# DonsetPG/graph-physics

Measured on AMD Instinct MI355X. Metric: training steps/sec, CylinderFlow 15-round MGN (batch 16 meshes per step), higher is better.
Workload: dtype f32; 1 GPU; BASELINE.json configs[1], fp32: 16 x 1885-node CylinderFlow-like meshes per GPU (N=30160, E=180082), 15 rounds, latent 128, random init; global_batch_meshes=16, launch=eager, parallelism=single

## Files before the change

graph-physics_amd/_capi.py:

```python
from __future__ import annotations

import ctypes as C
import os
import subprocess
import threading

_HERE = os.path.dirname(os.path.abspath(__file__))
_CSRC = os.path.join(_HERE, "csrc")
_REPO = os.path.dirname(_HERE)
LIB_PATH = os.environ.get("MGN_LIB") or os.path.join(_CSRC, "libmgn_hip.so")
SOURCES = [os.path.join(_CSRC, "mgn_kernels.hip"), os.path.join(_CSRC, "mgn_prep.hip"), os.path.join(_CSRC, "mgn_attn.hip"),
           os.path.join(_CSRC, "mgn_dense.hip"), os.path.join(_CSRC, "mgn_loss.hip"), os.path.join(_CSRC, "mgn_khop.hip"),
           os.path.join(_CSRC, "mgn_subgraph.hip"), os.path.join(_CSRC, "mgn_randedge.hip"), os.path.join(_CSRC, "mgn_knn.hip")]
DEPS = [os.path.join(_CSRC, "mgn_x6.inc"), os.path.join(_CSRC, "mgn_fused.inc"), os.path.join(_CSRC, "mgn_pp.inc"), os.path.join(_CSRC, "mgn_ppr.inc"),
        os.path.join(_CSRC, "mgn_philox.inc"), os.path.join(_CSRC, "mgn_host.inc"), os.path.join(_CSRC, "mgn_graphprim.inc"),
        os.path.join(_CSRC, "mgn_rollout.inc"), os.path.join(_CSRC, "mgn_starattn.inc"),
        os.path.join(_CSRC, "mgn_slice.inc")]
HEADER = os.path.join(_REPO, "include", "mgn_hip.h")
EXT_HEADER = os.path.join(_REPO, "include", "mgn_hip_ext.h")
MTP_HEADER = os.path.join(_REPO, "include", "mgn_hip_mtp.h")
SLICE_HEADER = os.path.join(_REPO, "include", "mgn_hip_slice.h")
DEVICE_FLAGS = ["-Xclang", "-target-feature", "-Xclang", "-packed-fp32-ops"]

MAX_LAYERS = 8
# ... 4 lines not shown
_i32p = C.c_void_p


class MlpFwdArgs(C.Structure):
    _fields_ = [
        ("M", C.c_int64),
        ("H", C.c_int), ("NL", C.c_int), ("nphase", C.c_int),
        ("src", _f32p * MAX_PHASES),
        ("idx", _i32p * MAX_PHASES),
        ("kw", C.c_int * MAX_PHASES),
        ("W", _f32p * MAX_LAYERS),
        ("b", _f32p * MAX_LAYERS),
        ("scale", _f32p),
        ("eps", C.c_float),
        ("out_w", C.c_int),
        ("resid", _f32p),
        ("out", _f32p),
        ("y_out", _f32p),
        ("saveH", _f32p * MAX_LAYERS),
        ("saveU", _f32p),
        ("saveR", _f32p),
        ("ldw0", C.c_int), ("n_add", C.c_int),
        ("add_src", _f32p * 2), ("add_idx", _i32p * 2),
        ("n_post", C.c_int), ("post_ldw", C.c_int),
        ("post_W", _f32p * 2), ("post_out", _f32p * 2),
        ("wpk", C.c_void_p * 8),
        ("saveM", C.c_void_p * MAX_LAYERS),
        ("precision", C.c_int),
        ("out_relu", C.c_int),
        ("seg_key", C.c_void_p), ("seg_rowptr", C.c_void_p), ("seg_out", _f32p), ("seg_part", _f32p),
        ("act", C.c_int),
        ("saveZ", _f32p * MAX_LAYERS),
        ("add_rows", C.c_int64 * 2),
    ]


class MlpBwdArgs(C.Structure):
    _fields_ = [
        ("M", C.c_int64),
        ("H", C.c_int), ("NL", C.c_int),
        ("dOut", _f32p),
        ("dOut2", _f32p),
        ("idx2", _i32p),
        ("out_w", C.c_int),
        ("U", _f32p), ("R", _f32p), ("scale", _f32p), ("eps", C.c_float),
        ("Hs", _f32p * MAX_LAYERS),
        ("WT", _f32p * MAX_LAYERS),
        ("dZ", _f32p * MAX_LAYERS),
        ("n_din", C.c_int),
        ("WT0", _f32p * MAX_PHASES),
        ("din_resid", _f32p * MAX_PHASES),
        ("dIn", _f32p * MAX_PHASES),
        ("db", _f32p * MAX_LAYERS),
        ("dscale", _f32p),
        ("red_ws", C.c_void_p), ("red_ws_bytes", C.c_size_t),
        ("wpk", C.c_void_p * 8),
        ("Ms", C.c_void_p * MAX_LAYERS),
        ("precision", C.c_int),
        ("n_front", C.c_int),
        ("front_src", _f32p * MAX_PHASES),
        ("front_resid", _f32p),
        ("front_out", _f32p),
        ("defer_reduce", C.c_int),
        ("act", C.c_int),
        ("Zs", _f32p * MAX_LAYERS),
        ("seg_key", C.c_void_p), ("seg_rowptr", C.c_void_p), ("seg_out", _f32p), ("seg_part", _f32p),
# ... 373 lines not shown
```

graph-physics_amd/csrc/mgn_kernels.hip:

```cpp
#include <hip/hip_runtime.h>
#include <stdint.h>
#include <stdlib.h>
#include <type_traits>
#include "mgn_hip.h"

typedef float f32x4 __attribute__((ext_vector_type(4)));

#define MFMA16(a, b, c) __builtin_amdgcn_mfma_f32_16x16x4f32((a), (b), (c), 0, 0, 0)

typedef __attribute__((address_space(1))) const f32x4 g_cf32x4;
typedef __attribute__((address_space(1))) f32x4 g_f32x4;
typedef __attribute__((address_space(1))) const float g_cfloat;
typedef __attribute__((address_space(1))) float g_float;
__device__ __forceinline__ f32x4 ld4(const float* p) { return *(g_cf32x4*)p; }
__device__ __forceinline__ void st4(float* p, f32x4 v) { *(g_f32x4*)p = v; }
__device__ __forceinline__ void st4_stream(float* p, f32x4 v) { *(g_f32x4*)p = v; }
__device__ __forceinline__ float ld1(const float* p) { return *(g_cfloat*)p; }
__device__ __forceinline__ void st1(float* p, float v) { *(g_float*)p = v; }

template <int HB, int MT>
__device__ __forceinline__ void gemm_tl(f32x4 (&acc)[MT][HB], const f32x4 (&in)[MT][HB],
                                        const float* __restrict__ W, int ldw, int nib, int nkb,
                                        int c, int g) {
  const float* wl = W + (size_t)c * ldw + 4 * g;
// ... 306 lines not shown
      for (int ib = 0; ib < HB; ++ib) acc[t][ib] = ld4(a.scale + 16 * ib + 4 * g) * in[t][ib];
    }
    if (a.saveU != nullptr) store_tl<HB, MT, RAGGED>(a.saveU, in, H, mm, valid, g);
  }
  if (a.y_out != nullptr) store_tl<HB, MT, RAGGED>(a.y_out, acc, a.out_w, mm, valid, g);
  if (a.resid != nullptr) {
    int nkb;
    load_tl<HB, MT, RAGGED>(in, a.resid, nullptr, a.out_w, mm, g, nkb);
#pragma unroll
    for (int t = 0; t < MT; ++t)
#pragma unroll
      for (int ib = 0; ib < HB; ++ib) acc[t][ib] = in[t][ib] + acc[t][ib];
  }
  if (a.out_relu) {
#pragma unroll
    for (int t = 0; t < MT; ++t)
#pragma unroll
      for (int ib = 0; ib < HB; ++ib)
#pragma unroll
        for (int r = 0; r < 4; ++r) acc[t][ib][r] = act_f(acc[t][ib][r], a.act);
    if (a.saveM[0] != nullptr) {
#pragma unroll
      for (int t = 0; t < MT; ++t) {
        uint32_t bits = 0;
#pragma unroll
        for (int ib = 0; ib < HB; ++ib)
#pragma unroll
          for (int r = 0; r < 4; ++r) bits |= (acc[t][ib][r] > 0.f) ? (1u << (4 * ib + r)) : 0u;
        if (valid[t]) a.saveM[0][mm[t] * 4 + g] = bits;
      }
    }
  }
  store_tl<HB, MT, RAGGED>(a.out, acc, a.out_w, mm, valid, g);
}

template <int HB, int MT>
__device__ __forceinline__ void colsum_to_lds(float* lds_w, const f32x4 (&v)[MT][HB], int c, int g) {
#pragma unroll
  for (int ib = 0; ib < HB; ++ib) {
    f32x4 s = v[0][ib];
#pragma unroll
    for (int t = 1; t < MT; ++t) s += v[t][ib];
#pragma unroll
    for (int r = 0; r < 4; ++r) s[r] = colsum16(s[r]);
    if (c == 0) *(f32x4*)(lds_w + 16 * ib + 4 * g) = s;
  }
}

template <int HB, int MT>
__device__ __forceinline__ void colsum_to_lds_add(float* lds_w, const f32x4 (&v)[MT][HB], int c, int g) {
#pragma unroll
  for (int ib = 0; ib < HB; ++ib) {
    f32x4 s = v[0][ib];
#pragma unroll
    for (int t = 1; t < MT; ++t) s += v[t][ib];
#pragma unroll
    for (int r = 0; r < 4; ++r) s[r] = colsum16(s[r]);
    if (c == 0) *(f32x4*)(lds_w + 16 * ib + 4 * g) += s;
  }
}

template <int HB, int MT, bool RAGGED>
__global__ void __launch_bounds__(256, (MT >= 4) ? 1 : 2) k_mlp_bwd(const mgn_mlp_bwd_args a) {
  constexpr int H = 16 * HB;
  __shared__ float lds[4 * (MGN_MAX_LAYERS + 1) * H];
  const int lane = threadIdx.x & 63, wv = threadIdx.x >> 6;
// ... 1742 lines not shown
  w.ppr_bwd = num("MGN_PPR_BWD", 1) != 0;
  w.nw = num("MGN_NW", 4);
  const int budget = num("MGN_WGRAD_GENERIC_BUDGET", 0);
  w.wgrad_generic_budget = (budget >= 64 && budget <= 1024) ? budget : 512;
  w.wgrad_no_row64 = set("MGN_WGRAD_NO_ROW64");
  w.wgrad_pc = num("MGN_WGRAD_PC", 1) != 0;
  w.wgrad_no_interleave = set("MGN_WGRAD_NO_INTERLEAVE");
  w.wgrad_row64_exact = set("MGN_WGRAD_ROW64_EXACT");
  return w;
}

enum KernelSig { SIG_FWD, SIG_BWD, SIG_BWD_PPR, SIG_WGRAD, SIG_COUNT };
struct KernelRow {
  const char* name;
  const void* fn;
  int sig;
  int lds;
};
#define KROW(sig, type, lds, ...) {#__VA_ARGS__, (const void*)static_cast<type>(__VA_ARGS__), sig, lds}
#define FWD(lds, ...) KROW(SIG_FWD, void (*)(mgn_mlp_fwd_args), lds, __VA_ARGS__)
#define BWD(lds, ...) KROW(SIG_BWD, void (*)(mgn_mlp_bwd_args), lds, __VA_ARGS__)
#define BWD_PPR(lds, ...) KROW(SIG_BWD_PPR, void (*)(mgn_mlp_bwd_args, int), lds, __VA_ARGS__)
#define WGRAD(lds, ...) KROW(SIG_WGRAD, void (*)(WgradLaunch), lds, __VA_ARGS__)
#define GEN_LDS_RESERVE (2 * WBUF_BYTES + 4 * 7 * 128 * 4)
#define X6_BWD_RESERVE X6_BWD_LDS_BYTES(LDS_MAX_NL + 1)
#define GENERIC_ROWS(ROW, k)                                                                                                      \
  ROW(0, k<8,2,true>), ROW(0, k<8,1,true>), ROW(0, k<8,2,false>), ROW(0, k<8,1,false>), ROW(0, k<4,2,true>), ROW(0, k<4,1,true>), \
  ROW(0, k<4,2,false>), ROW(0, k<4,1,false>), ROW(0, k<2,2,true>), ROW(0, k<2,1,true>), ROW(0, k<2,2,false>), ROW(0, k<2,1,false>), \
  ROW(0, k<1,2,true>), ROW(0, k<1,1,true>), ROW(0, k<1,2,false>), ROW(0, k<1,1,false>)
enum Kernel {
  K_FWD_PPR = 0, K_FWD_PP = 4, K_FWD_NW6 = 6, K_FWD_EDGE = 7, K_FWD_NODE2 = 9, K_FWD_NODE0 = 11, K_FWD_SILU = 13, K_FWD_NW8_BF16 = 15,
  K_FWD_LDS = 16, K_FWD_GEN = 18, K_BWD_FRONT = 34, K_BWD_SILU = 36, K_BWD_SEG = 38, K_BWD_EDGE = 39, K_BWD_PPR = 41, K_BWD_LDS = 43,
  K_BWD_GEN = 45, K_WGRAD_X6 = 61, K_WGRAD_ROW64_BF16 = 63, K_WGRAD_ROW64X6 = 67, K_WGRAD_ROW64 = 69, K_WGRAD_GEN = 70, K_WGRAD_RED = 74,
  K_FWD_DYN = 76, K_FWD_NW8 = 78, K_BWD_DYN = 79, K_WGRAD_LDS = 81, K_WGRAD_PC = 82, K_COUNT = 83
};
static const KernelRow kKernels[] = {
    FWD(PPR_LDS_BYTES, k_edge_fwd_ppr<true,true>), FWD(PPR_LDS_BYTES, k_edge_fwd_ppr<false,true>),
    FWD(PPR_LDS_BYTES, k_edge_fwd_ppr<true,false>), FWD(PPR_LDS_BYTES, k_edge_fwd_ppr<false,false>),
    FWD(PP_LDS_BYTES, k_edge_fwd_pp<true>), FWD(PP_LDS_BYTES, k_edge_fwd_pp<false>),
    FWD(X6_FWD_LDS_BYTES(6), k_mlp_fwd_x6<6,6,0,ShEdge>),
    FWD(X6_FWD_LDS_BYTES(4), k_mlp_fwd_x6<1,4,0,ShEdge>), FWD(X6_FWD_LDS_BYTES(4), k_mlp_fwd_x6<6,4,0,ShEdge>),
    FWD(X6_FWD_LDS_BYTES(4), k_mlp_fwd_x6<1,4,0,ShNode<2>>), FWD(X6_FWD_LDS_BYTES(4), k_mlp_fwd_x6<6,4,0,ShNode<2>>),
    FWD(X6_FWD_LDS_BYTES(4), k_mlp_fwd_x6<1,4,0,ShNode<0>>), FWD(X6_FWD_LDS_BYTES(4), k_mlp_fwd_x6<6,4,0,ShNode<0>>),
    FWD(X6_FWD_LDS_BYTES(4), k_mlp_fwd_x6<1,4,1>), FWD(X6_FWD_LDS_BYTES(4), k_mlp_fwd_x6<6,4,1>),
    FWD(X6_FWD_LDS_BYTES(8), k_mlp_fwd_x6<1,8,0>),
    FWD(GEN_LDS_RESERVE, k_mlp_fwd_lds<2>), FWD(GEN_LDS_RESERVE, k_mlp_fwd_lds<1>),
    GENERIC_ROWS(FWD, k_mlp_fwd),
    BWD(X6_BWD_RESERVE, k_mlp_bwd_x6<6,true,0>), BWD(X6_BWD_RESERVE, k_mlp_bwd_x6<1,true,0>),
    BWD(X6_BWD_RESERVE, k_mlp_bwd_x6<6,false,1>), BWD(X6_BWD_RESERVE, k_mlp_bwd_x6<1,false,1>),
    BWD(X6_BWD_RESERVE, k_mlp_bwd_x6<6,false,0,true>),
    BWD(X6_BWD_RESERVE, k_mlp_bwd_x6<6,false,0,false,SbEdge>), BWD(X6_BWD_RESERVE, k_mlp_bwd_x6<1,false,0,false,SbEdge>),
    BWD_PPR(PPB_LDS_BYTES, k_edge_bwd_ppr<true>), BWD_PPR(PPB_LDS_BYTES, k_edge_bwd_ppr<false>),
    BWD(GEN_LDS_RESERVE, k_mlp_bwd_lds<2>), BWD(GEN_LDS_RESERVE, k_mlp_bwd_lds<1>),
    GENERIC_ROWS(BWD, k_mlp_bwd),
    WGRAD(4 * WG_TILE_BYTES, k_wgrad_x6<6>), WGRAD(4 * WG_TILE_BYTES, k_wgrad_x6<1>),
    WGRAD(0, k_wgrad_row64<true,true,true>), WGRAD(0, k_wgrad_row64<true,true,false>), WGRAD(0, k_wgrad_row64<true,false,true>),
    WGRAD(0, k_wgrad_row64<true>),
    WGRAD(0, k_wgrad_row64x6<true>), WGRAD(0, k_wgrad_row64x6<false>), WGRAD(0, k_wgrad_row64<false>),
    WGRAD(0, k_wgrad<8>), WGRAD(0, k_wgrad<4>), WGRAD(0, k_wgrad<2>), WGRAD(0, k_wgrad<1>),
    WGRAD(0, k_wgrad_red<4>), WGRAD(0, k_wgrad_red<16>),
    FWD(X6_FWD_LDS_BYTES(4), k_mlp_fwd_x6<6,4,0>), FWD(X6_FWD_LDS_BYTES(4), k_mlp_fwd_x6<1,4,0>), FWD(X6_FWD_LDS_BYTES(8), k_mlp_fwd_x6<6,8,0>),
    BWD(X6_BWD_RESERVE, k_mlp_bwd_x6<6,false,0>), BWD(X6_BWD_RESERVE, k_mlp_bwd_x6<1,false,0>),
    WGRAD(4 * WG_TILE_BYTES, k_wgrad_lds), WGRAD(WPC_LDS_BYTES, k_wgrad_pc),
};
static_assert(sizeof(kKernels) / sizeof(kKernels[0]) == K_COUNT, "kKernels and enum Kernel disagree");
#undef GENERIC_ROWS
#undef WGRAD
#undef BWD_PPR
#undef BWD
#undef FWD
#undef KROW

static int reserve_lds(int k) {
  static thread_local bool done[SIG_COUNT];
  const int sig = kKernels[k].sig;
  if (kKernels[k].lds == 0 || done[sig]) return 0;
  for (const KernelRow& r : kKernels)
    if (r.sig == sig && r.lds > 0 && hipFuncSetAttribute(r.fn, hipFuncAttributeMaxDynamicSharedMemorySize, r.lds) != hipSuccess) return 1;
  done[sig] = true;
  return 0;
}
template <class... A>
static void launch(int k, dim3 grid, unsigned block, size_t lds, hipStream_t s, const A&... args) {
  void* argv[] = {(void*)&args...};
  (void)hipLaunchKernel(kKernels[k].fn, grid, dim3(block), argv, lds, s);
}

struct MlpPlan {
  bool lds;
  bool lds_shape;
  int mt;
  unsigned grid;
  size_t smem;
};
static MlpPlan plan_mlp(const Switches& w, int64_t M, int H, int NL, bool ragged, bool bwd, int act) {
  MlpPlan p;
// ... 43 lines not shown
  if (a.seg_out != nullptr && (a.seg_key == nullptr || a.seg_rowptr == nullptr || a.seg_part == nullptr || a.n_post > 0)) return false;
  for (int u = 0; u < G; ++u)
    if (a.wpk[u] == nullptr) return false;
  return true;
}
static int fwd_static_shape(const mgn_mlp_fwd_args& a, const Switches& w) {
  if (w.x6_static == 0 || a.act != MGN_ACT_RELU || a.NL != 4 || a.resid == nullptr || a.scale == nullptr) return 0;
  if (a.nphase == 1 && a.n_add == 2 && a.n_post == 0 && a.idx[0] == nullptr && a.add_idx[0] != nullptr && a.add_idx[1] != nullptr &&
      a.seg_out != nullptr && a.seg_key == a.add_idx[0])
    return 1;
  if (w.x6_static != 2 && a.nphase == 2 && a.n_add == 0 && a.idx[0] == nullptr && a.idx[1] == nullptr && a.seg_out == nullptr && a.M >= 4 * 512 * 64)
    return a.n_post == 2 ? 2 : a.n_post == 0 ? 3 : 0;
  return 0;
}
static bool fwd_edge_stream_ok(const mgn_mlp_fwd_args& a, int64_t min_rows) {
  return a.precision == 0 && a.y_out == nullptr && a.M >= min_rows && a.M * 512 < (int64_t)1 << 32 && units_back_to_back(a.wpk) &&
         fwd_saves(a) >= 0 && a.resid != nullptr && a.scale != nullptr && a.out != a.resid && a.out != a.src[0];
}
static bool fwd_pp_ok(const mgn_mlp_fwd_args& a, const Switches& w) {
  if (w.pp == 0 || (w.pp < 0 && fwd_saves(a) != 0)) return false;
  return fwd_edge_stream_ok(a, w.pp == 2 ? 1 : 2 * 128 * 256);
}
static bool fwd_ppr_ok(const mgn_mlp_fwd_args& a, const Switches& w) {
  if (w.ppr == 0) return false;
  for (int q = 0; q < 2; ++q)
    if (a.add_rows[q] <= 0 || a.add_rows[q] * 512 >= (int64_t)1 << 32) return false;
  return fwd_edge_stream_ok(a, w.ppr == 2 ? 1 : 65536);
}
static unsigned ppr_groups(int64_t M) {
  const int64_t ngroups = ((M + 15) / 16 + PPR_R - 1) / PPR_R;
  return (ngroups < 256) ? (unsigned)ngroups : 256u;
}

static MlpRoute route_fwd(const mgn_mlp_fwd_args& a, const Switches& w) {
  bool ragged = (a.out_w != a.H) || a.nphase > MGN_MAX_PHASES;
  for (int p = 0; p < a.nphase && p < MGN_MAX_PHASES; ++p) ragged = ragged || (a.kw[p] != a.H);
  const MlpPlan p = plan_mlp(w, a.M, a.H, a.NL, ragged, false, a.act);
  MlpRoute r;
  r.lds_path = p.lds;
  r.lds_shape = p.lds_shape;
  r.x6 = fwd_x6(a, w);
  r.grid = p.grid;
  r.block = 256;
  r.lds = p.smem;
  r.nblocks = 0;
  if (!p.lds) {
    r.kernel = K_FWD_GEN + generic_row(a.H, ragged, p.mt);
    return r;
  }
  if (!r.x6) {
    r.kernel = K_FWD_LDS + (p.mt == 2 ? 0 : 1);
    return r;
  }
  const bool silu = (a.act == MGN_ACT_SILU);
  const int nw = (w.nw == 8 && a.seg_out == nullptr && !silu) ? 8 : 4;
  const bool nw6 = (w.nw == 6);
  const int fp32 = (a.precision >= 1) ? 0 : 1;
  const int rows = 16 * nw;
  r.grid = (unsigned)((a.M + rows - 1) / rows);
  const unsigned cap = (nw == 8) ? 256u : 512u;
  if (r.grid > cap) r.grid = cap;
  if (w.grid > 0 && (unsigned)w.grid < r.grid) r.grid = (unsigned)w.grid;
  r.block = 64 * nw;
  r.lds = X6_FWD_LDS_BYTES(nw);
  const int shape = (nw == 4 && !silu) ? fwd_static_shape(a, w) : 0;
  if (shape == 1 && !nw6 && fwd_ppr_ok(a, w)) {
    r.kernel = K_FWD_PPR + (a.saveU != nullptr ? 0 : 1) + (w.ppr_xcd ? 0 : 2);
    r.grid = ppr_groups(a.M);
    r.block = 512;
    r.lds = PPR_LDS_BYTES;
  } else if (shape == 1 && !nw6 && fwd_pp_ok(a, w)) {
    r.kernel = K_FWD_PP + (a.saveU != nullptr ? 0 : 1);
    r.grid = (unsigned)((a.M + 127) / 128);
    if (r.grid > 256u) r.grid = 256u;
    r.block = 512;
    r.lds = PP_LDS_BYTES;
  } else if (shape == 1 && nw6 && a.precision == 0) {
    r.kernel = K_FWD_NW6;
// ... 79 lines not shown
    r.kernel = K_BWD_PPR + (w.ppr_xcd ? 0 : 1);
    r.grid = ppr_groups(a.M);
    if (r.grid > p.grid) r.grid = p.grid;
    r.block = 512;
    r.lds = PPB_LDS_BYTES;
  } else if (sb_edge) {
    r.kernel = K_BWD_EDGE + bf16;
  } else if (a.seg_out != nullptr) {
    r.kernel = K_BWD_SEG;
  } else if (a.act == MGN_ACT_SILU) {
    r.kernel = K_BWD_SILU + bf16;
  } else {
    r.kernel = (front ? K_BWD_FRONT : K_BWD_DYN) + bf16;
  }
  return r;
}

extern "C" {

static int check_mlp_common(int H, int NL, int out_w, const char* who) {
  if (!(H == 16 || H == 32 || H == 64 || H == 128)) return fail(1, "H must be 16, 32, 64 or 128");
  if (NL < 1 || NL > MGN_MAX_LAYERS) return fail(1, "NL out of range");
  if (out_w < 1 || out_w > H) return fail(1, "out_w out of range");
  (void)who;
  return 0;
}


int mgn_mlp_fwd(const mgn_mlp_fwd_args* args, void* stream) {
  const mgn_mlp_fwd_args& a = *args;
  if (int rc = check_mlp_common(a.H, a.NL, a.out_w, "mgn_mlp_fwd")) return rc;
  const Switches w = read_switches();
  const MlpRoute r = route_fwd(a, w);
  if (a.precision < 0 || a.precision > 2) return fail(1, "mgn_mlp_fwd: precision must be 0 (fp32-grade), 1 (bf16) or 2 (bf16, two-byte saves)");
  if (a.precision == 2 && (!r.x6 || !r.lds_path || a.act != MGN_ACT_RELU))
    return fail(1, "mgn_mlp_fwd: precision 2 (two-byte saves) needs the packed split-bf16 path (H = 128, wpk[]) and ReLU");
  if (a.seg_out != nullptr && !(r.lds_shape && r.x6))
    return fail(1, "mgn_mlp_fwd: the fused segment sum needs the packed split-bf16 path (and seg_key / seg_rowptr / seg_part, no post-products)");
  if (a.out_relu && (a.scale != nullptr || a.resid != nullptr || a.wpk[0] != nullptr || r.lds_shape))
    return fail(1, "mgn_mlp_fwd: out_relu is for a plain ragged-input launch (no norm / residual / packed path)");
  if (a.act != MGN_ACT_RELU && a.act != MGN_ACT_SILU && a.act != MGN_ACT_GELU) return fail(1, "mgn_mlp_fwd: act must be MGN_ACT_RELU, _SILU or _GELU");
  if (a.act == MGN_ACT_GELU && (a.wpk[0] != nullptr || a.precision != 0 || a.seg_out != nullptr || a.n_add > 0 || a.n_post > 0 || a.ldw0 > 0))
    return fail(1, "mgn_mlp_fwd: GELU runs on the generic kernels only (no packed weights / gathers / post-products)");
  if (a.act == MGN_ACT_SILU && r.lds_shape && !r.x6 && a.NL > 1)
    return fail(1, "mgn_mlp_fwd: SiLU is not available on the exact-fp32 LDS generation (pass packed weights)");
  if (a.precision >= 1 && r.lds_path && !r.x6)
    return fail(1, "mgn_mlp_fwd: at H = 128 with full widths the bf16 matrix mode needs the packed split-bf16 path (wpk); other shapes run it on the generic kernels");
  if (a.nphase < 1 || a.nphase > MGN_MAX_PHASES) return fail(1, "mgn_mlp_fwd: nphase out of range");
  for (int p = 0; p < a.nphase; ++p)
    if (a.kw[p] < 1 || a.kw[p] > a.H) return fail(1, "mgn_mlp_fwd: phase width out of range");
  if (a.scale != nullptr && a.out_w != a.H) return fail(1, "mgn_mlp_fwd: RMSNorm needs out_w == H");
  if (a.n_add < 0 || a.n_add > 2 || a.n_post < 0 || a.n_post > 2) return fail(1, "mgn_mlp_fwd: n_add / n_post out of range");
  if ((a.n_add > 0 || a.n_post > 0 || a.ldw0 > 0) && !r.lds_shape)
    return fail(1, "mgn_mlp_fwd: ldw0 / n_add / n_post need the H = 128 full-width kernel");
  if (a.M == 0) return 0;
  if (reserve_lds(r.kernel)) return fail(2, "mgn_mlp_fwd: cannot reserve LDS");
  launch(r.kernel, dim3(r.grid), r.block, r.lds, (hipStream_t)stream, a);
  return check_launch("mgn_mlp_fwd");
}


size_t mgn_mlp_bwd_workspace_bytes(int64_t M, int H, int NL) {
  return (size_t)((M + 63) / 64 + 1) * (NL + 1) * H * sizeof(float);
}


// ... 279 lines not shown
```

graph-physics_amd/csrc/mgn_prep.hip:

```cpp
#include "mgn_hip.h"
#include "mgn_host.inc"
#include "mgn_graphprim.inc"

extern "C" const char* mgn_prep_last_error(void) { return g_err; }

__global__ void k_face_keys(const int64_t* __restrict__ face, int K, long F, long N, uint64_t* __restrict__ keys, int* __restrict__ err) {
  const long f = (long)blockIdx.x * blockDim.x + threadIdx.x;
  if (f >= F) return;
  int64_t v[4];
  bool ok = true;
  for (int k = 0; k < K; ++k) {
    v[k] = face[(size_t)k * F + f];
    ok = ok && v[k] >= 0 && v[k] < N;
  }
  if (!ok) *err = 1;
  const int npair = K * (K - 1) / 2;
  int p = 0;
  for (int a = 0; a < K; ++a)
    for (int b = a + 1; b < K; ++b, ++p) {
      const bool keep = ok && v[a] != v[b];
      keys[(size_t)p * F + f] = keep ? edge_key(v[a], v[b], N) : EDGE_KEY_DROPPED;
      keys[(size_t)(npair + p) * F + f] = keep ? edge_key(v[b], v[a], N) : EDGE_KEY_DROPPED;
    }
}
// ... 292 lines not shown

extern "C" int mgn_edge_features(const float* pos, int D, const int64_t* src, const int64_t* dst, int64_t E, float* edge_attr, void* stream) {
  hipStream_t s = (hipStream_t)stream;
  if (D != 2 && D != 3) return fail(1, "mgn_edge_features: positions must be 2-D or 3-D");
  if (E <= 0) return 0;
  const unsigned grid = (unsigned)((E + 255) / 256);
  if (D == 2)
    hipLaunchKernelGGL(k_edge_features<2>, dim3(grid), dim3(256), 0, s, pos, src, dst, (long)E, edge_attr);
  else
    hipLaunchKernelGGL(k_edge_features<3>, dim3(grid), dim3(256), 0, s, pos, src, dst, (long)E, edge_attr);
  return check_launch("mgn_edge_features");
}

#define SIM_MAXW 32
#define SIM_PART 256

__device__ __forceinline__ float sim_value(const mgn_sim_desc& d, int stream, long row, int col) {
  if (stream == 0) {
    const int nf = d.feat_end - d.feat_start;
    if (col < nf) return d.x[row * d.x_w + d.feat_start + col];
    const float t = d.x[row * d.x_w + d.type_idx];
    const int ti = (int)(long)t;
    if (col == nf && d.type_err != nullptr && (ti < 0 || ti >= MGN_NODE_TYPES)) *d.type_err = 1;
    return (ti == col - nf) ? 1.f : 0.f;
  }
  if (stream == 1) return d.y[row * d.y_w + col] - d.x[row * d.x_w + d.out_start + col];
  return d.edge_attr[row * d.edge_w + col];
}
__device__ __forceinline__ int sim_width(const mgn_sim_desc& d, int stream) {
  return stream == 0 ? (d.feat_end - d.feat_start) + MGN_NODE_TYPES : stream == 1 ? d.out_w : d.edge_w;
}
__device__ __forceinline__ long sim_rows(const mgn_sim_desc& d, int stream) { return stream == 2 ? d.E : d.N; }

__global__ void __launch_bounds__(256) k_stats_partial(const mgn_sim_desc d, float* __restrict__ part) {
  const int stream = blockIdx.y;
  if (!d.accumulate[stream] || !(*d.num_acc[stream] < d.max_accumulations)) return;
  const int W = sim_width(d, stream);
  const long M = sim_rows(d, stream);
  __shared__ float s1[256], s2[256];
  const int col = threadIdx.x % SIM_MAXW, rl = threadIdx.x / SIM_MAXW;
  float a = 0.f, b = 0.f;
  if (col < W)
    for (long r = (long)blockIdx.x * 8 + rl; r < M; r += (long)SIM_PART * 8) {
      const float v = sim_value(d, stream, r, col);
      a += v;
      b = fmaf(v, v, b);
    }
  s1[threadIdx.x] = a;
  s2[threadIdx.x] = b;
  __syncthreads();
  if (rl == 0) {
    for (int k = 1; k < 8; ++k) {
      a += s1[k * SIM_MAXW + col];
      b += s2[k * SIM_MAXW + col];
    }
    float* p = part + ((size_t)(stream * SIM_PART + blockIdx.x) * 2) * SIM_MAXW;
    p[col] = a;
    p[SIM_MAXW + col] = b;
  }
}

__global__ void __launch_bounds__(64) k_stats_final(const mgn_sim_desc d, const float* __restrict__ part) {
  const int stream = blockIdx.x;
  if (!d.accumulate[stream] || !(*d.num_acc[stream] < d.max_accumulations)) return;
  const int W = sim_width(d, stream);
  const int col = threadIdx.x % SIM_MAXW, which = threadIdx.x / SIM_MAXW;
  if (col < W) {
    float t = 0.f;
    for (int b = 0; b < SIM_PART; ++b) t += part[((size_t)(stream * SIM_PART + b) * 2 + which) * SIM_MAXW + col];
    float* dst = which == 0 ? d.acc_sum[stream] : d.acc_sumsq[stream];
    dst[col] += t;
  }
  if (threadIdx.x == 0) {
    *d.acc_count[stream] += (float)sim_rows(d, stream);
    *d.num_acc[stream] += 1.f;
  }
}

__global__ void __launch_bounds__(256) k_sim_normalize(const mgn_sim_desc d) {
  const int stream = blockIdx.y;
// ... 656 lines not shown
```

graph-physics_amd/ops.py:

```python
from __future__ import annotations

import ctypes as C
from typing import List, Optional, Sequence, Tuple

import torch

from . import _capi
from ._launch import call, ptr as _ptr, stream as _stream, stream_object, workspace

EPS = 1e-8
import os as _os
X6_ENABLED = _os.environ.get("MGN_FP32_MFMA") is None

_matrix_precision = "fp32"


def set_matrix_precision(p: str) -> None:
    global _matrix_precision
    if p not in ("fp32", "bf16"):
        raise ValueError("matrix precision must be 'fp32' or 'bf16'")
    if p == "bf16" and not X6_ENABLED:
        raise RuntimeError("bf16 matrix mode runs on the split-bf16 kernels; unset MGN_FP32_MFMA")
    _matrix_precision = p

# ... 257 lines not shown

def segsum(src: torch.Tensor, rowptr: torch.Tensor, perm: Optional[torch.Tensor], out: Optional[torch.Tensor] = None) -> torch.Tensor:
    _require_device(src)
    n = rowptr.numel() - 1
    H = src.shape[1]
    if not src.is_contiguous():
        raise ValueError("segsum: src must be contiguous rows (a column slice of a wider tensor is not)")
    if out is None:
        out = torch.empty(n, H, dtype=torch.float32, device=src.device)
    call("mgn_segsum", src.device, _ptr(src), _ptr(rowptr), _ptr(perm), _ptr(out), n, H)
    return out


def seg_fix(rowptr: torch.Tensor, part: torch.Tensor, out: torch.Tensor):
    call("mgn_seg_fix", out.device, _ptr(rowptr), _ptr(part), _ptr(out), rowptr.numel() - 1)


def segsum2(src: torch.Tensor, rowptr0, perm0, out0, rowptr1, perm1, out1):
    n = rowptr0.numel() - 1
    if not src.is_contiguous():
        raise ValueError("segsum2: src must be contiguous rows (a column slice of a wider tensor is not)")
    name = "mgn_segsum2_b16" if src.dtype == torch.bfloat16 else "mgn_segsum2"
    call(name, src.device, _ptr(src), _ptr(rowptr0), _ptr(perm0), _ptr(out0), _ptr(rowptr1), _ptr(perm1), _ptr(out1), n, src.shape[1])


def mlp_fwd(M: int, H: int, phases: Sequence[Tuple[torch.Tensor, Optional[torch.Tensor], int]],
            Ws: Sequence[torch.Tensor], bs: Sequence[Optional[torch.Tensor]], scale: Optional[torch.Tensor],
            out_w: int, resid: Optional[torch.Tensor], out: torch.Tensor, y_out: Optional[torch.Tensor] = None,
            saveH: Optional[Sequence[torch.Tensor]] = None, saveU: Optional[torch.Tensor] = None,
            saveR: Optional[torch.Tensor] = None, ldw0: int = 0,
            adds: Sequence[Tuple[torch.Tensor, Optional[torch.Tensor]]] = (),
            posts: Sequence[Tuple[int, torch.Tensor]] = (), post_ldw: int = 0, wpk: Sequence[int] = (),
            saveM: Optional[Sequence[torch.Tensor]] = None, precision: int = 0, out_relu: bool = False,
            seg=None, act: int = 0, saveZ: Optional[Sequence[torch.Tensor]] = None):
    a = _capi.MlpFwdArgs()
    a.M, a.H, a.NL, a.nphase = M, H, len(Ws), len(phases)
    for p, (src, idx, kw) in enumerate(phases):
        a.src[p], a.idx[p], a.kw[p] = _ptr(src), _ptr(idx), kw
    for l, (W, b) in enumerate(zip(Ws, bs)):
        a.W[l], a.b[l] = _ptr(W), _ptr(b)
    a.scale, a.eps, a.out_w = _ptr(scale), EPS, out_w
    a.resid, a.out, a.y_out = _ptr(resid), _ptr(out), _ptr(y_out)
    if saveH is not None:
        for l, h in enumerate(saveH):
            a.saveH[l] = _ptr(h)
    a.saveU, a.saveR = _ptr(saveU), _ptr(saveR)
    a.ldw0, a.n_add, a.n_post, a.post_ldw = ldw0, len(adds), len(posts), post_ldw
    for q, (t, ix) in enumerate(adds):
        a.add_src[q], a.add_idx[q], a.add_rows[q] = _ptr(t), _ptr(ix), t.shape[0]
    for q, (wptr, o) in enumerate(posts):
        a.post_W[q], a.post_out[q] = wptr, _ptr(o)
    for u, addr in enumerate(wpk):
        a.wpk[u] = addr
    if saveM is not None:
        for l, t in enumerate(saveM):
            a.saveM[l] = _ptr(t)
    a.precision = precision
    a.out_relu = int(out_relu)
    if seg is not None:
        a.seg_key, a.seg_rowptr, a.seg_out, a.seg_part = (_ptr(t) for t in seg)
    a.act = act
    if saveZ is not None:
        for l, t in enumerate(saveZ):
            a.saveZ[l] = _ptr(t)
    call("mgn_mlp_fwd", out.device, C.byref(a))


def mlp_bwd(M: int, H: int, NL: int, dOut: torch.Tensor, dOut2, idx2, out_w: int, U, R, scale,
            Hs: Sequence[torch.Tensor], WT: Sequence[Optional[torch.Tensor]], dZ: Sequence[Optional[torch.Tensor]],
            din: Sequence[Tuple[torch.Tensor, Optional[torch.Tensor], torch.Tensor]],
            db: Sequence[Optional[torch.Tensor]], dscale: Optional[torch.Tensor], wpk: Sequence[int] = (),
            Ms: Optional[Sequence[torch.Tensor]] = None, precision: int = 0, front=None, defer: Optional[list] = None,
            act: int = 0, Zs: Optional[Sequence[torch.Tensor]] = None, seg=None):
    L = _capi.lib()
    a = _capi.MlpBwdArgs()
    a.M, a.H, a.NL = M, H, NL
    a.dOut, a.dOut2, a.idx2, a.out_w = _ptr(dOut), _ptr(dOut2), _ptr(idx2), out_w
    a.dOut2_rows = dOut2.shape[0] if dOut2 is not None else 0
    a.U, a.R, a.scale, a.eps = _ptr(U), _ptr(R), _ptr(scale), EPS
    for l, h in enumerate(Hs or ()):
        a.Hs[l] = _ptr(h)
    for l in range(NL):
        a.WT[l] = _ptr(WT[l])
        a.dZ[l] = _ptr(dZ[l])
        a.db[l] = _ptr(db[l])
    a.n_din = len(din)
    for q, (wt0, res, dst) in enumerate(din):
        a.WT0[q], a.din_resid[q], a.dIn[q] = _ptr(wt0), _ptr(res), _ptr(dst)
    a.dscale = _ptr(dscale)
    for u, addr in enumerate(wpk):
        a.wpk[u] = addr
    if Ms is not None:
        for l, t in enumerate(Ms):
            a.Ms[l] = _ptr(t)
    a.precision = precision
    a.act = act
    if Zs is not None:
# ... 275 lines not shown
        dev = x.device
        kp, op = pad16(kin), pad16(out_w)
        W0 = Ws[0]
        if kp != kin:
            W0 = torch.nn.functional.pad(W0, (0, kp - kin))
        Wl, bl = Ws[-1], bs[-1]
        if op != out_w:
            Wl = torch.nn.functional.pad(Wl, (0, 0, 0, op - out_w))
            bl = torch.nn.functional.pad(bl, (0, op - out_w))
        Wk = [W0] + Ws[1:-1] + [Wl]
        bk = bs[:-1] + [bl]
        prec = 1 if (_matrix_precision == "bf16" and not (H == 128 and out_w == H and X6_ENABLED and act != 2)) else 0
        if prec:
            Wk = [w.to(torch.bfloat16).to(torch.float32) for w in Wk]
            bk = [b.to(torch.bfloat16).to(torch.float32) for b in bk]
        need = any(ctx.needs_input_grad) and _saving()
        f = dict(dtype=torch.float32, device=dev)
        y = torch.empty(M, out_w, **f)
        x6 = H == 128 and out_w == H and X6_ENABLED and M > 0 and act != 2
        mode = "generic"
        if x6 and kin < H and 3 <= NL <= 4:
            mode = "enc"
        elif x6 and kin == H and NL <= 4:
            mode = "full"
        packed = mode != "generic"
        saveH = [torch.empty(M, H, **f) for _ in range(NL - 1)] if need else None
        U = torch.empty(M, H, **f) if (need and has_norm) else None
        R = torch.empty(M, **f) if (need and has_norm) else None
        Ms = [torch.empty(M, 4, dtype=torch.int32, device=dev) for _ in range(NL - 1)] if (need and packed and act == 0) else None
        Zs = [torch.empty(M, H, **f) for _ in range(NL - 1)] if (need and act != 0) else None
        if mode == "enc":
            h1 = saveH[0] if need else torch.empty(M, H, **f)
            mlp_fwd(M, H, [(x, None, kin)], [Wk[0]], [bk[0]], None, H, None, h1, Zs[0] if Zs else None, out_relu=True, act=act,
                    saveM=[Ms[0]] if Ms else None)
            pk = torch.empty((NL - 1) * _capi.WPACK_BYTES, dtype=torch.uint8, device=dev)
            units = [pk.data_ptr() + u * _capi.WPACK_BYTES for u in range(NL - 1)]
            wpack([(Wk[l + 1].data_ptr(), H, False, units[l]) for l in range(NL - 1)], dev)
            mlp_fwd(M, H, [(h1, None, H)], Wk[1:], bk[1:], scale, out_w, None, y, None,
                    saveH[1:] if need else None, U, R, wpk=units, saveM=Ms[1:] if Ms else None,
                    saveZ=Zs[1:] if Zs else None, act=act)
        elif mode == "full":
            pk = torch.empty(NL * _capi.WPACK_BYTES, dtype=torch.uint8, device=dev)
            units = [pk.data_ptr() + u * _capi.WPACK_BYTES for u in range(NL)]
            wpack([(Wk[l].data_ptr(), H, False, units[l]) for l in range(NL)], dev)
            mlp_fwd(M, H, [(x, None, H)], Wk, bk, scale, out_w, None, y, None, saveH, U, R, wpk=units, saveM=Ms, saveZ=Zs, act=act)
        elif M > 0:
            mlp_fwd(M, H, [(x, None, kin)], Wk, bk, scale, out_w, None, y, None, saveH, U, R, act=act, saveZ=Zs, precision=prec)
        ctx.meta = (NL, H, kin, out_w, has_norm, kp != kin, op != out_w, act, mode)
        ctx.prec, ctx.Wk_rounded = prec, (Wk if prec else None)
        ctx.save_for_backward(x, *Ws, *([scale] if has_norm else []))
        ctx.pads = (W0 if kp != kin else None, Wl if op != out_w else None)
        ctx.saved_acts = (saveH, U, R, Ms, Zs)
        return y

    @staticmethod
    def backward(ctx, dy):
        NL, H, kin, out_w, has_norm, pad0, padl, act, mode = ctx.meta
        if ctx.saved_acts is None or ctx.saved_acts[0] is None:
            raise RuntimeError("MlpFunction: no saved activations -- backward ran a second time without retain_graph "
                               "support, or the forward ran under no_grad")
        t = ctx.saved_tensors
        x, Ws = t[0], list(t[1:1 + NL])
        scale = t[1 + NL] if has_norm else None
        Wk = [ctx.pads[0] if pad0 else Ws[0]] + Ws[1:-1] + [ctx.pads[1] if padl else Ws[-1]]
        prec = getattr(ctx, "prec", 0)
        if prec:
            Wk = ctx.Wk_rounded
# ... 566 lines not shown
```

include/mgn_hip.h:

```cpp
#ifndef MGN_HIP_H
#define MGN_HIP_H

#include <stddef.h>
#include <stdint.h>

#ifdef __cplusplus
extern "C" {
#endif

#define MGN_MAX_LAYERS 8
#define MGN_MAX_PHASES 3
#define MGN_MAX_WGRAD_JOBS 48

int mgn_version(void);
const char* mgn_last_error(void);

size_t mgn_csr_workspace_bytes(int64_t E, int64_t N);
int mgn_csr_build(const int64_t* key, int64_t E, int64_t N, int32_t* rowptr, int32_t* perm,
                  void* ws, size_t ws_bytes, void* stream);

size_t mgn_topology_workspace_bytes(int64_t E, int64_t N);
int mgn_topology_build(const int64_t* src, const int64_t* dst, int64_t E, int64_t N, int32_t* rowptr_dst, int32_t* perm_dst,
                       int32_t* src_s, int32_t* dst_s, int32_t* rowptr_src, int32_t* perm_src, int32_t* max_degree_host,
                       void* ws, size_t ws_bytes, void* stream);
// ... 17 lines not shown
  const float* src[MGN_MAX_PHASES];
  const int32_t* idx[MGN_MAX_PHASES];
  int kw[MGN_MAX_PHASES];
  const float* W[MGN_MAX_LAYERS];
  const float* b[MGN_MAX_LAYERS];
  const float* scale;
  float eps;
  int out_w;
  const float* resid;
  float* out;
  float* y_out;
  float* saveH[MGN_MAX_LAYERS];
  float* saveU;
  float* saveR;
  int ldw0;
  int n_add;
  const float* add_src[2];
  const int32_t* add_idx[2];
  int n_post;
  int post_ldw;
  const float* post_W[2];
  float* post_out[2];
  const void* wpk[8];
  uint32_t* saveM[MGN_MAX_LAYERS];
  int precision;
  int out_relu;
  const int32_t* seg_key;
  const int32_t* seg_rowptr;
  float* seg_out;
  float* seg_part;
  int act;
  float* saveZ[MGN_MAX_LAYERS];
  int64_t add_rows[2];
} mgn_mlp_fwd_args;
#define MGN_ACT_RELU 0
#define MGN_ACT_SILU 1
#define MGN_ACT_GELU 2
int mgn_mlp_fwd(const mgn_mlp_fwd_args* args, void* stream);

typedef struct {
  int64_t M;
  int H, NL;
  const float* dOut;
  const float* dOut2;
  const int32_t* idx2;
  int out_w;
  const float* U; const float* R; const float* scale; float eps;
  const float* Hs[MGN_MAX_LAYERS];
  const float* WT[MGN_MAX_LAYERS];
  float* dZ[MGN_MAX_LAYERS];
  int n_din;
  const float* WT0[MGN_MAX_PHASES];
  const float* din_resid[MGN_MAX_PHASES];
  float* dIn[MGN_MAX_PHASES];
  float* db[MGN_MAX_LAYERS];
  float* dscale;
  void* red_ws; size_t red_ws_bytes;
  const void* wpk[8];
  const uint32_t* Ms[MGN_MAX_LAYERS];
  int precision;
  int n_front;
  const float* front_src[MGN_MAX_PHASES];
  const float* front_resid;
  float* front_out;
  int defer_reduce;
  int act;
// ... 319 lines not shown
```

Before: 82.48 steps/s.

## Add row-stream kernel for narrow encoder first layer and prefetch stats loads

Adds a dedicated kernel for the encoder's first linear layer when the input width is at most 4. Each lane keeps its four output columns of weights in registers and streams rows with a one-step prefetch, writing the ReLU output and a ballot-packed activation mask. This replaces the generic MFMA path, which pads the tiny K dimension. The normalization statistics kernel is also rewritten to issue 32 strided loads ahead before accumulating, and it now checks node-type range inline.

```diff
diff --git a/graph-physics_amd/_capi.py b/graph-physics_amd/_capi.py
--- a/graph-physics_amd/_capi.py
+++ b/graph-physics_amd/_capi.py
@@ -60,6 +60,7 @@
         ("act", C.c_int),
         ("saveZ", _f32p * MAX_LAYERS),
         ("add_rows", C.c_int64 * 2),
+        ("variant", C.c_int32),
     ]
 
 
diff --git a/graph-physics_amd/csrc/mgn_kernels.hip b/graph-physics_amd/csrc/mgn_kernels.hip
--- a/graph-physics_amd/csrc/mgn_kernels.hip
+++ b/graph-physics_amd/csrc/mgn_kernels.hip
@@ -362,6 +362,74 @@
     }
   }
   store_tl<HB, MT, RAGGED>(a.out, acc, a.out_w, mm, valid, g);
+}
+
+#define RS_ROWS_PER_WAVE 8
+#define RS_ROWS_PER_WG (4 * RS_ROWS_PER_WAVE)
+#define RS_MAX_GRID 1024
+#define RS_KB 4
+__device__ __forceinline__ void first_rows_load(float (&xin)[RS_ROWS_PER_WAVE / 2][RS_KB], const float* __restrict__ x, long base, int half,
+                                                long M, int kw) {
+#pragma unroll
+  for (int t = 0; t < RS_ROWS_PER_WAVE / 2; ++t) {
+    const long m = base + 2 * t + half;
+    const float* p = x + (m < M ? m : M - 1) * kw;
+#pragma unroll
+    for (int k = 0; k < RS_KB; ++k) xin[t][k] = ld1(p + (k < kw ? k : kw - 1));
+  }
+}
+__global__ void __launch_bounds__(256) k_first_rows(const mgn_mlp_fwd_args a) {
+  const int lane = threadIdx.x & 63, wv = threadIdx.x >> 6;
+  const int j = lane & 31, half = lane >> 5;
+  const int kw = a.kw[0];
+  float w[4][RS_KB];
+#pragma unroll
+  for (int q = 0; q < 4; ++q) {
+    const f32x4 t = ld4(a.W[0] + (size_t)(4 * j + q) * 16);
+#pragma unroll
+    for (int r = 0; r < 4; ++r) w[q][r] = t[r];
+  }
+  f32x4 bias = {0.f, 0.f, 0.f, 0.f};
+  if (a.b[0] != nullptr) bias = ld4(a.b[0] + 4 * j);
+  const float* __restrict__ x = a.src[0];
+  const long stride = (long)gridDim.x * RS_ROWS_PER_WG;
+  long base = (long)blockIdx.x * RS_ROWS_PER_WG + wv * RS_ROWS_PER_WAVE;
+  float xin[RS_ROWS_PER_WAVE / 2][RS_KB], xnext[RS_ROWS_PER_WAVE / 2][RS_KB];
+  first_rows_load(xin, x, base, half, a.M, kw);
+  for (; base < a.M; base += stride) {
+    first_rows_load(xnext, x, base + stride, half, a.M, kw);
+#pragma unroll
+    for (int t = 0; t < RS_ROWS_PER_WAVE / 2; ++t) {
+      const long m = base + 2 * t + half;
+      const bool valid = m < a.M;
+      f32x4 z = bias;
+#pragma unroll
+      for (int k = 0; k < RS_KB; ++k)
+        if (k < kw) {
+#pragma unroll
+          for (int q = 0; q < 4; ++q) z[q] = fmaf(w[q][k], xin[t][k], z[q]);
+        }
+      if (a.y_out != nullptr && valid) st4(a.y_out + m * 128 + 4 * j, z);
+      f32x4 h;
+#pragma unroll
+      for (int q = 0; q < 4; ++q) h[q] = act_f(z[q], a.act);
+      if (a.saveM[0] != nullptr) {
+        uint32_t word = 0;
+#pragma unroll
+        for (int q = 0; q < 4; ++q) {
+          const unsigned long long bal = __ballot(h[q] > 0.f);
+          const uint32_t mine = (uint32_t)(bal >> (32 * half));
+          word |= ((mine >> (j & 3)) & 0x11111111u) << q;
+        }
+        if (valid && j < 4) st1((float*)(a.saveM[0] + m * 4 + j), __builtin_bit_cast(float, word));
+      }
+      if (valid) st4(a.out + m * 128 + 4 * j, h);
+    }
+#pragma unroll
+    for (int t = 0; t < RS_ROWS_PER_WAVE / 2; ++t)
+#pragma unroll
+      for (int k = 0; k < RS_KB; ++k) xin[t][k] = xnext[t][k];
+  }
 }
 
 template <int HB, int MT>
@@ -2170,7 +2238,7 @@
   K_FWD_PPR = 0, K_FWD_PP = 4, K_FWD_NW6 = 6, K_FWD_EDGE = 7, K_FWD_NODE2 = 9, K_FWD_NODE0 = 11, K_FWD_SILU = 13, K_FWD_NW8_BF16 = 15,
   K_FWD_LDS = 16, K_FWD_GEN = 18, K_BWD_FRONT = 34, K_BWD_SILU = 36, K_BWD_SEG = 38, K_BWD_EDGE = 39, K_BWD_PPR = 41, K_BWD_LDS = 43,
   K_BWD_GEN = 45, K_WGRAD_X6 = 61, K_WGRAD_ROW64_BF16 = 63, K_WGRAD_ROW64X6 = 67, K_WGRAD_ROW64 = 69, K_WGRAD_GEN = 70, K_WGRAD_RED = 74,
-  K_FWD_DYN = 76, K_FWD_NW8 = 78, K_BWD_DYN = 79, K_WGRAD_LDS = 81, K_WGRAD_PC = 82, K_COUNT = 83
+  K_FWD_DYN = 76, K_FWD_NW8 = 78, K_BWD_DYN = 79, K_WGRAD_LDS = 81, K_WGRAD_PC = 82, K_FWD_ROWS = 83, K_COUNT = 84
 };
 static const KernelRow kKernels[] = {
     FWD(PPR_LDS_BYTES, k_edge_fwd_ppr<true,true>), FWD(PPR_LDS_BYTES, k_edge_fwd_ppr<false,true>),
@@ -2200,6 +2268,7 @@
     FWD(X6_FWD_LDS_BYTES(4), k_mlp_fwd_x6<6,4,0>), FWD(X6_FWD_LDS_BYTES(4), k_mlp_fwd_x6<1,4,0>), FWD(X6_FWD_LDS_BYTES(8), k_mlp_fwd_x6<6,8,0>),
     BWD(X6_BWD_RESERVE, k_mlp_bwd_x6<6,false,0>), BWD(X6_BWD_RESERVE, k_mlp_bwd_x6<1,false,0>),
     WGRAD(4 * WG_TILE_BYTES, k_wgrad_lds), WGRAD(WPC_LDS_BYTES, k_wgrad_pc),
+    FWD(0, k_first_rows),
 };
 static_assert(sizeof(kKernels) / sizeof(kKernels[0]) == K_COUNT, "kKernels and enum Kernel disagree");
 #undef GENERIC_ROWS
@@ -2309,6 +2378,12 @@
   return (ngroups < 256) ? (unsigned)ngroups : 256u;
 }
 
+static bool fwd_first_rows_ok(const mgn_mlp_fwd_args& a) {
+  return a.H == 128 && a.NL == 1 && a.nphase == 1 && a.kw[0] >= 1 && a.kw[0] <= RS_KB && a.idx[0] == nullptr && a.out_w == 128 && a.out_relu &&
+         a.precision == 0 && a.scale == nullptr && a.resid == nullptr && a.wpk[0] == nullptr && a.ldw0 == 0 && a.n_add == 0 && a.n_post == 0 &&
+         a.seg_out == nullptr && a.saveH[0] == nullptr && a.saveU == nullptr && a.saveR == nullptr && a.M >= 1;
+}
+
 static MlpRoute route_fwd(const mgn_mlp_fwd_args& a, const Switches& w) {
   bool ragged = (a.out_w != a.H) || a.nphase > MGN_MAX_PHASES;
   for (int p = 0; p < a.nphase && p < MGN_MAX_PHASES; ++p) ragged = ragged || (a.kw[p] != a.H);
@@ -2321,6 +2396,12 @@
   r.block = 256;
   r.lds = p.smem;
   r.nblocks = 0;
+  if (a.variant == 1 && fwd_first_rows_ok(a)) {
+    r.kernel = K_FWD_ROWS;
+    const int64_t groups = (a.M + RS_ROWS_PER_WG - 1) / RS_ROWS_PER_WG;
+    r.grid = groups < RS_MAX_GRID ? (unsigned)groups : (unsigned)RS_MAX_GRID;
+    return r;
+  }
   if (!p.lds) {
     r.kernel = K_FWD_GEN + generic_row(a.H, ragged, p.mt);
     return r;
@@ -2466,6 +2547,7 @@
   if (int rc = check_mlp_common(a.H, a.NL, a.out_w, "mgn_mlp_fwd")) return rc;
   const Switches w = read_switches();
   const MlpRoute r = route_fwd(a, w);
+  if (a.variant != 0 && a.variant != 1) return fail(1, "mgn_mlp_fwd: variant must be 0 or 1 (the row-stream narrow first layer)");
   if (a.precision < 0 || a.precision > 2) return fail(1, "mgn_mlp_fwd: precision must be 0 (fp32-grade), 1 (bf16) or 2 (bf16, two-byte saves)");
   if (a.precision == 2 && (!r.x6 || !r.lds_path || a.act != MGN_ACT_RELU))
     return fail(1, "mgn_mlp_fwd: precision 2 (two-byte saves) needs the packed split-bf16 path (H = 128, wpk[]) and ReLU");
diff --git a/graph-physics_amd/csrc/mgn_prep.hip b/graph-physics_amd/csrc/mgn_prep.hip
--- a/graph-physics_amd/csrc/mgn_prep.hip
+++ b/graph-physics_amd/csrc/mgn_prep.hip
@@ -348,6 +348,7 @@
 }
 __device__ __forceinline__ long sim_rows(const mgn_sim_desc& d, int stream) { return stream == 2 ? d.E : d.N; }
 
+#define SIM_AHEAD 32
 __global__ void __launch_bounds__(256) k_stats_partial(const mgn_sim_desc d, float* __restrict__ part) {
   const int stream = blockIdx.y;
   if (!d.accumulate[stream] || !(*d.num_acc[stream] < d.max_accumulations)) return;
@@ -356,12 +357,37 @@
   __shared__ float s1[256], s2[256];
   const int col = threadIdx.x % SIM_MAXW, rl = threadIdx.x / SIM_MAXW;
   float a = 0.f, b = 0.f;
-  if (col < W)
-    for (long r = (long)blockIdx.x * 8 + rl; r < M; r += (long)SIM_PART * 8) {
-      const float v = sim_value(d, stream, r, col);
-      a += v;
-      b = fmaf(v, v, b);
-    }
+  if (col < W) {
+    const int nf = d.feat_end - d.feat_start;
+    const bool hot = stream == 0 && col >= nf, two = stream == 1;
+    const float* pa = stream == 0 ? d.x + (hot ? d.type_idx : d.feat_start + col) : stream == 1 ? d.y + col : d.edge_attr + col;
+    const float* pb = d.x + d.out_start + col;
+    const long sa = stream == 0 ? d.x_w : stream == 1 ? d.y_w : d.edge_w, sb = d.x_w;
+    const long step = (long)SIM_PART * 8;
+    bool bad = false;
+    for (long r0 = (long)blockIdx.x * 8 + rl; r0 < M; r0 += SIM_AHEAD * step) {
+      float va[SIM_AHEAD], vb[SIM_AHEAD];
+#pragma unroll
+      for (int k = 0; k < SIM_AHEAD; ++k) {
+        const long r = r0 + k * step, rc = r < M ? r : M - 1;
+        va[k] = pa[rc * sa];
+        vb[k] = two ? pb[rc * sb] : 0.f;
+      }
+#pragma unroll
+      for (int k = 0; k < SIM_AHEAD; ++k)
+        if (r0 + k * step < M) {
+          float v = two ? va[k] - vb[k] : va[k];
+          if (hot) {
+            const int ti = (int)(long)va[k];
+            if (col == nf && (ti < 0 || ti >= MGN_NODE_TYPES)) bad = true;
+            v = (ti == col - nf) ? 1.f : 0.f;
+          }
+          a += v;
+          b = fmaf(v, v, b);
+        }
+    }
+    if (bad && d.type_err != nullptr) *d.type_err = 1;
+  }
   s1[threadIdx.x] = a;
   s2[threadIdx.x] = b;
   __syncthreads();
diff --git a/graph-physics_amd/ops.py b/graph-physics_amd/ops.py
--- a/graph-physics_amd/ops.py
+++ b/graph-physics_amd/ops.py
@@ -313,7 +313,7 @@
             adds: Sequence[Tuple[torch.Tensor, Optional[torch.Tensor]]] = (),
             posts: Sequence[Tuple[int, torch.Tensor]] = (), post_ldw: int = 0, wpk: Sequence[int] = (),
             saveM: Optional[Sequence[torch.Tensor]] = None, precision: int = 0, out_relu: bool = False,
-            seg=None, act: int = 0, saveZ: Optional[Sequence[torch.Tensor]] = None):
+            seg=None, act: int = 0, saveZ: Optional[Sequence[torch.Tensor]] = None, variant: int = 0):
     a = _capi.MlpFwdArgs()
     a.M, a.H, a.NL, a.nphase = M, H, len(Ws), len(phases)
     for p, (src, idx, kw) in enumerate(phases):
@@ -344,6 +344,7 @@
     if saveZ is not None:
         for l, t in enumerate(saveZ):
             a.saveZ[l] = _ptr(t)
+    a.variant = variant
     call("mgn_mlp_fwd", out.device, C.byref(a))
 
 
@@ -685,7 +686,7 @@
         if mode == "enc":
             h1 = saveH[0] if need else torch.empty(M, H, **f)
             mlp_fwd(M, H, [(x, None, kin)], [Wk[0]], [bk[0]], None, H, None, h1, Zs[0] if Zs else None, out_relu=True, act=act,
-                    saveM=[Ms[0]] if Ms else None)
+                    saveM=[Ms[0]] if Ms else None, variant=1)
             pk = torch.empty((NL - 1) * _capi.WPACK_BYTES, dtype=torch.uint8, device=dev)
             units = [pk.data_ptr() + u * _capi.WPACK_BYTES for u in range(NL - 1)]
             wpack([(Wk[l + 1].data_ptr(), H, False, units[l]) for l in range(NL - 1)], dev)
diff --git a/include/mgn_hip.h b/include/mgn_hip.h
--- a/include/mgn_hip.h
+++ b/include/mgn_hip.h
@@ -73,6 +73,7 @@
   int act;
   float* saveZ[MGN_MAX_LAYERS];
   int64_t add_rows[2];
+  int32_t variant;
 } mgn_mlp_fwd_args;
 #define MGN_ACT_RELU 0
 #define MGN_ACT_SILU 1
```

Result: no change. 83.03 steps/s, median of 3 (+0.7%).
